# clementinboittiaux/sucre

Hardware: AMD Instinct MI355X
Metric: restored Mpixels/sec/GPU at 1080p, 64 neighbour views; % HBM roofline (higher is better)
Workload: dtype f32

## Files before the change

### sucre_amd/csrc/fit.hip

```cpp
#include <cstddef>
#include <type_traits>

#include "experiment.h"
#include "fit_math.h"
#include "handoff.h"

namespace sucre {

struct Water {
    float B[3], nb[3], ng[3];
};

template <class ParamAt>
__device__ __forceinline__ Water water_from(ParamAt param_at) {
    Water w;
#pragma unroll
    for (int c = 0; c < 3; ++c) {
        w.B[c] = param_at(c);
        w.nb[c] = -param_at(3 + c) * kLog2e;
        w.ng[c] = -param_at(6 + c) * kLog2e;
    }
    return w;
}
__device__ __forceinline__ Water load_water(const float *__restrict__ params) {
// ... 32 lines not shown
#pragma unroll
        for (int c = 0; c < 3; ++c) { e.a[j][c] = zz[j] * w.nb[c]; e.g[j][c] = zz[j] * w.ng[c]; }
    __builtin_amdgcn_sched_barrier(0);
#pragma unroll
    for (int j = 0; j < kGroupLv; ++j)
#pragma unroll
        for (int c = 0; c < 3; ++c) { e.a[j][c] = fast_exp2(e.a[j][c]); e.g[j][c] = fast_exp2(e.g[j][c]); }
    __builtin_amdgcn_sched_barrier(0);
}

__device__ __forceinline__ void grad_terms(float z, float a, float g, uint32_t k, bool valid, float Bc, float Jc, int c, Acc &acc) {
    const float omg = 1.0f - g;
    const float Ihat = __builtin_fmaf(Jc, a, Bc * omg);
    float r = __builtin_fmaf((float)k, kInv255, -Ihat);
    r = valid ? r : 0.0f;
    const float rz = r * z;
    acc.cost = __builtin_fmaf(r, r, acc.cost);
    acc.pa[c] = __builtin_fmaf(r, a, acc.pa[c]);
    acc.pb[c] = __builtin_fmaf(rz, a, acc.pb[c]);
    acc.sB[c] = __builtin_fmaf(r, omg, acc.sB[c]);
    acc.sGZ[c] = __builtin_fmaf(rz, g, acc.sGZ[c]);
}

template <bool kMasked>
__device__ __forceinline__ void accumulate_chunk(const float (&zz)[kGroupLv], const uint32_t (&cc)[3], const Water &w,
                                                 const float (&J)[3], Acc &acc) {
    if (kExpNoCompute) {
        acc.cost += (zz[0] + zz[1]) + (zz[2] + zz[3]) + (float)(cc[0] ^ cc[1] ^ cc[2]);
        return;
    }
    Exps e;
    chunk_exps(zz, w, e);
#pragma unroll
    for (int j = 0; j < kGroupLv; ++j) {
        const float z = zz[j];
        const bool valid = !kMasked || z > 0.0f;
#pragma unroll
        for (int c = 0; c < 3; ++c) grad_terms(z, e.a[j][c], e.g[j][c], (cc[c] >> (8 * j)) & 255u, valid, w.B[c], J[c], c, acc);
    }
}

__device__ __forceinline__ void accumulate_level(float z, const uint32_t (&k)[3], const Water &w, const float (&J)[3],
                                                 Acc &acc) {
    const bool valid = z > 0.0f;
#pragma unroll
    for (int c = 0; c < 3; ++c) grad_terms(z, fast_exp2(z * w.nb[c]), fast_exp2(z * w.ng[c]), k[c], valid, w.B[c], J[c], c, acc);
}

__device__ __forceinline__ float finite_or_zero(float x) { return __builtin_isfinite(x) ? x : 0.0f; }

struct AccOne {
    float q[9][3];
};

__device__ __forceinline__ void closed_terms(float z, float a, float g, uint32_t k, bool valid, float Bc, float Jp,
                                             float &q0, float &q1, float &q2, float &q3, float &q4, float &q5,
                                             float &q6, float &q7, float &q8) {
    const float omg = 1.0f - g;
    const float y = __builtin_fmaf((float)k, kInv255, -(Bc * omg));
    float p = __builtin_fmaf(-Jp, a, y);
    p = valid ? p : 0.0f;
    const float za = z * a, zg = z * g;
    q0 = __builtin_fmaf(p, a, q0);
    q1 = __builtin_fmaf(a, valid ? a : 0.0f, q1);
    q2 = __builtin_fmaf(p, omg, q2);
    q3 = __builtin_fmaf(a, omg, q3);
    q4 = __builtin_fmaf(p, za, q4);
    q5 = __builtin_fmaf(a, za, q5);
    q6 = __builtin_fmaf(p, zg, q6);
    q7 = __builtin_fmaf(a, zg, q7);
    q8 = __builtin_fmaf(p, p, q8);
}

template <bool kMasked>
__device__ __forceinline__ void accumulate_chunk(const float (&zz)[kGroupLv], const uint32_t (&cc)[3], const Water &w,
                                                 const float (&Jp)[3], AccOne &acc) {
    if (kExpNoCompute) {
        acc.q[8][0] += (zz[0] + zz[1]) + (zz[2] + zz[3]) + (float)(cc[0] ^ cc[1] ^ cc[2]);
        return;
    }
    Exps e;
    chunk_exps(zz, w, e);
#pragma unroll
    for (int j = 0; j < kGroupLv; ++j) {
        const float z = zz[j];
        const bool valid = !kMasked || z > 0.0f;
#pragma unroll
        for (int c = 0; c < 3; ++c)
            closed_terms(z, e.a[j][c], e.g[j][c], (cc[c] >> (8 * j)) & 255u, valid, w.B[c], Jp[c], acc.q[0][c], acc.q[1][c],
                         acc.q[2][c], acc.q[3][c], acc.q[4][c], acc.q[5][c], acc.q[6][c], acc.q[7][c], acc.q[8][c]);
    }
}

__device__ __forceinline__ void accumulate_level(float z, const uint32_t (&k)[3], const Water &w, const float (&Jp)[3],
                                                 AccOne &acc) {
    if (kExpNoCompute) {
        acc.q[8][0] += z + (float)(k[0] ^ k[1] ^ k[2]);
        return;
    }
    const bool valid = z > 0.0f;
#pragma unroll
    for (int c = 0; c < 3; ++c)
        closed_terms(z, fast_exp2(z * w.nb[c]), fast_exp2(z * w.ng[c]), k[c], valid, w.B[c], Jp[c], acc.q[0][c], acc.q[1][c],
                     acc.q[2][c], acc.q[3][c], acc.q[4][c], acc.q[5][c], acc.q[6][c], acc.q[7][c], acc.q[8][c]);
}

constexpr int kRing = SUCRE_RING;
constexpr int kAhead = kRing - 1;
constexpr int kSlot = 2048;

struct __attribute__((aligned(16))) FitLds {
    uint8_t ring[4][kRing][kSlot];
    double stot[kSumsPad];
    float wsum[4][kNumSums];
    double wtotal[4][kNumSums];
    int is_last, is_last_total;
};

__device__ __forceinline__ uint32_t lds_addr(const void *p) {
    return static_cast<uint32_t>(reinterpret_cast<uintptr_t>(p));
}

constexpr uint32_t kShapeFull = 1u << 31;
constexpr uint32_t kShapeTrail = 1u << 30;
__host__ __device__ constexpr uint32_t full_chunk_b(int fmt) { return (uint32_t)(chunk_bytes(fmt) - 1024) / 16u; }
__host__ __device__ __forceinline__ uint32_t item_shape(uint32_t bytes, bool full_chunk) {
    const uint32_t pieces = bytes / 16u;
// ... 12 lines not shown
        "s_mov_b32 %0, m0\n\t"
        "s_mov_b32 m0, %3\n\t"
        "s_nop 0\n\t"
        "global_load_lds_dwordx4 %1, %2" SUCRE_DMA_POLICY "\n\t"
        "s_mov_b32 m0, %4\n\t"
        "s_nop 0\n\t"
        "global_load_lds_dwordx4 %5, %2" SUCRE_DMA_POLICY "\n\t"
        "s_mov_b32 m0, %0"
        : "=&s"(keep)
        : "v"(voffA), "s"(src), "s"(slotA), "s"(slotB), "v"(voffB)
        : "memory");
}

__device__ __forceinline__ void wait_vm(uint32_t n) {
#define SUCRE_W(N) case N: asm volatile("s_waitcnt vmcnt(" #N ")" ::: "memory"); break;
    switch (n) {
        SUCRE_W(0) SUCRE_W(1) SUCRE_W(2) SUCRE_W(3) SUCRE_W(4) SUCRE_W(5) SUCRE_W(6) SUCRE_W(7) SUCRE_W(8) SUCRE_W(9)
        SUCRE_W(10) SUCRE_W(11) SUCRE_W(12) SUCRE_W(13) SUCRE_W(14) SUCRE_W(15) SUCRE_W(16) SUCRE_W(17) SUCRE_W(18)
        SUCRE_W(19) SUCRE_W(20) SUCRE_W(21)
        default: asm volatile("s_waitcnt vmcnt(0)" ::: "memory"); break;
    }
#undef SUCRE_W
}
static_assert(2 * kAhead + 9 <= 63, "s_waitcnt vmcnt takes six bits");

__device__ __forceinline__ uint32_t strip_items(uint32_t levels, int mode) { return 1u + ((levels + 3u) >> 2) + (mode == 0 ? 1u : 0u); }

__global__ __launch_bounds__(256) void plan_kernel(const StripMeta *__restrict__ meta, int n_strips, const uint32_t *__restrict__ store_fmt, uint32_t W0, uint32_t W1,
                                                   uint32_t Kmax, uint32_t stride0, uint32_t stride1, uint32_t kmax0, uint32_t kmax1,
                                                   PlanItem *__restrict__ plan0, PlanItem *__restrict__ plan1,
                                                   StripEntry *__restrict__ strips0, StripEntry *__restrict__ strips1,
                                                   uint32_t *__restrict__ count0, uint32_t *__restrict__ count1, uint64_t comp_off,
                                                   uint64_t state_off) {
    const int mode = blockIdx.y;
    const int fmt = (int)store_fmt[0];
    const uint32_t W = mode ? W1 : W0, stride = mode ? stride1 : stride0, kmax = mode ? kmax1 : kmax0;
    PlanItem *plan = mode ? plan1 : plan0;
    StripEntry *strips = mode ? strips1 : strips0;
    uint32_t *count = mode ? count1 : count0;
    const uint32_t idx = blockIdx.x * 256u + threadIdx.x;
    const uint32_t wid = idx / Kmax, k = idx - wid * Kmax;
    if (wid >= W) return;
    const DealShares sh = deal_shares(mode, W / 4u);
    uint32_t start = 0u, strip = 0u, strip0 = 0u;
    const uint32_t K = deal_walk(wid, W, (uint32_t)n_strips, sh, [&](uint32_t s) { return meta[s].levels; }, [&](uint32_t kk, uint32_t s) {
        if (kk == 0u) strip0 = s;
        if (kk < k) start += strip_items(meta[s].levels, mode);
        if (kk == k) strip = s;
    });
    if (k == 0u) count[wid] = K;
    if (k >= K) return;
    const StripMeta m = meta[strip];
    const uint32_t nfull = m.levels >> 2, r = m.levels & 3u;
    const uint32_t nu = min(nfull, m.full >> 2);
    const uint32_t lb = (uint32_t)level_bytes(fmt);
    const uint64_t st = state_off + (uint64_t)strip * (kStateFloats * 4);
    PlanItem *out = plan + (size_t)wid * stride + start;
    strips[(size_t)wid * kmax + k] = StripEntry{strip, strip_counts(nu, nfull - nu, r)};
    *out++ = PlanItem{(uint32_t)(st >> 6), item_shape(3u * kStripPx * 4u, false)};
    for (uint32_t g = 0; g < nfull; ++g)
        *out++ = PlanItem{(uint32_t)((comp_off + (m.lvoff + (uint64_t)g * kGroupLv) * lb) >> 6), item_shape((uint32_t)chunk_bytes(fmt), true)};
    if (r) *out++ = PlanItem{(uint32_t)((comp_off + (m.lvoff + (uint64_t)nfull * kGroupLv) * lb) >> 6), item_shape(r * lb, false)};
    if (mode == 0) *out++ = PlanItem{(uint32_t)((st + 3 * kStripPx * 4) >> 6), item_shape(6u * kStripPx * 4u, false)};
    if (k + 1u == K) {
        const uint64_t st0 = state_off + (uint64_t)strip0 * (kStateFloats * 4);
        for (int j = 0; j < kAhead + 1; ++j) *out++ = PlanItem{(uint32_t)(st0 >> 6), item_shape(3u * kStripPx * 4u, false) | kShapeTrail};
    }
}

typedef uint32_t ItemRegs __attribute__((ext_vector_type(2)));
typedef const __attribute__((address_space(4))) ItemRegs *ConstItems;

template <class T>
__device__ __forceinline__ T *uniform_ptr(T *p) {
    const uint64_t u = reinterpret_cast<uint64_t>(p);
    const uint32_t lo = __builtin_amdgcn_readfirstlane((uint32_t)u), hi = __builtin_amdgcn_readfirstlane((uint32_t)(u >> 32));
    return reinterpret_cast<T *>(((uint64_t)hi << 32) | lo);
}

template <class T>
__device__ __forceinline__ ConstItems const_items(const T *p) {
    static_assert(sizeof(T) == 8, "two dwords per entry");
    return (ConstItems)(reinterpret_cast<uintptr_t>(uniform_ptr(p)));
}

struct RangeCodes { bool z24, z26; uint32_t zoff, fullB; };

template <int kFmt>
__device__ __forceinline__ RangeCodes range_codes_of(uint32_t f0, uint32_t f1) {
// ... 32 lines not shown
            asm("v_mad_u32_u24 %0, %1, 1, %2" : "=v"(bits) : "v"(w[j]), "s"(rc.zoff));
            if (kZ26) bits += ((h >> (2 * j)) & 3u) << 24;
            zz[j] = __uint_as_float(bits);
            if (masked) zz[j] = (kZ26 ? bits != rc.zoff : (w[j] & 0xffffffu) != 0u) ? zz[j] : 0.0f;
        }
        cc[0] = __builtin_amdgcn_perm(a.y, a.x, 0x0c0c0703u) | __builtin_amdgcn_perm(b.y, b.x, 0x07030c0cu);
        cc[1] = c.x; cc[2] = c.y;
    };
    if (kFmt == 0 && rc.z26) return read_codes(std::true_type{});
    if (kFmt == 0 && rc.z24) return read_codes(std::false_type{});
    if (kFmt == 0) {
        const float4 z4 = *reinterpret_cast<const float4 *>(sp + lane * 16);
        zz[0] = z4.x; zz[1] = z4.y; zz[2] = z4.z; zz[3] = z4.w;
    } else {
        const uint2 q = *reinterpret_cast<const uint2 *>(sp + lane * 8);
        zz[0] = (float)(q.x & 0xffffu) * kMPerMm; zz[1] = (float)(q.x >> 16) * kMPerMm;
        zz[2] = (float)(q.y & 0xffffu) * kMPerMm; zz[3] = (float)(q.y >> 16) * kMPerMm;
    }
    const uint32_t *cp = reinterpret_cast<const uint32_t *>(sp + (kFmt ? 2 : 4) * kStripPx * kGroupLv) + 3 * lane;
    cc[0] = cp[0]; cc[1] = cp[1]; cc[2] = cp[2];
}

template <int kFmt>
__device__ __forceinline__ void read_level(const uint8_t *sp, int lane, uint32_t r, uint32_t j, float &z, uint32_t (&k)[3], const RangeCodes &rc) {
    const bool z24 = kFmt == 0 && (rc.z24 || rc.z26);
    if (z24) {
        const uint8_t *zp = sp + (lane * r + j) * 3u;
        uint32_t code = (uint32_t)zp[0] | ((uint32_t)zp[1] << 8) | ((uint32_t)zp[2] << 16);
        if (rc.z26) {
            const uint32_t f = (uint32_t)lane * r + j;
            code |= ((reinterpret_cast<const uint32_t *>(sp + 6u * kStripPx * r)[f >> 4] >> (2u * (f & 15u))) & 3u) << 24;
        }
        z = code ? __uint_as_float(code + rc.zoff) : 0.0f;
    } else if (kFmt == 0) z = reinterpret_cast<const float *>(sp)[lane * r + j];
    else z = (float)reinterpret_cast<const uint16_t *>(sp)[lane * r + j] * kMPerMm;
    const uint8_t *cb = sp + (z24 ? 3 : kFmt ? 2 : 4) * kStripPx * r;
#pragma unroll
    for (int c = 0; c < 3; ++c) k[c] = cb[c * kStripPx * r + lane * r + j];
}

template <int kFmt>
__device__ __forceinline__ void issue_item(const ItemRegs it, uint32_t ring0, uint32_t slot_off, const uint8_t *__restrict__ ws, int lane, uint32_t fullB) {
    const uint32_t lane16 = (uint32_t)lane * 16u;
    const uint32_t voffB_full = (64u + min((uint32_t)lane, fullB - 1u)) * 16u;
    const uint8_t *src = ws + ((uint64_t)it.x << 6);
    const uint32_t slot = ring0 + slot_off;
    if (it.y & kShapeFull) {
        dma_item(src, slot, slot + 1024u, lane16, voffB_full);
    } else {
        const uint32_t a_last = it.y & 127u, b_last = (it.y >> 8) & 127u, b_base = (it.y >> 16) & 127u;
        dma_item(src, slot, slot + ((a_last + 1u) << 4), min((uint32_t)lane, a_last) << 4, (b_base + min((uint32_t)lane, b_last)) << 4);
    }
}

struct NoChain { static constexpr bool kOn = false; };
struct StreamChain {
    static constexpr bool kOn = true;
    ItemRegs head[kAhead + 1], se0;
    bool next_on;
    ItemRegs next_head[kAhead];
    const uint8_t *next_ws;
// ... 182 lines not shown
                if (kStep && t < 64) water_step(lds.stot, pstate, n_obs_total, co, trace_row);
            }
        }
    }
}

template <bool kFused, bool kStep = kFused>
__device__ __forceinline__ void finish_launch(FitLds &lds, float (&s)[kNumSums], float *partials, const AdamCoef &co,
                                              unsigned *ticket, double *gpart, int n_groups, double *sums,
                                              float *pstate, const uint64_t *__restrict__ n_obs_total,
                                              double *trace_row) {
    const int t = threadIdx.x;
    const int lane = t & 63;
    const int wave = __builtin_amdgcn_readfirstlane(t >> 6);
    wave_sums(s);
    if (lane == 0) {
#pragma unroll
        for (int q = 0; q < kNumSums; ++q) lds.wsum[wave][q] = s[q];
    }
    finish_from_wave_sums<kFused, kStep>(lds, partials, co, ticket, gpart, n_groups, sums, pstate, n_obs_total, trace_row);
}

template <class Chain>
__device__ __forceinline__ void store_stepped(float *p, float v) {
    if (kStoreNt == 1 || (kStoreNt == 2 && Chain::kOn)) __builtin_nontemporal_store(v, p);
    else *p = v;
}

template <int kFmt, bool kPrimed = false, class Chain = NoChain>
__device__ __forceinline__ void grad_pass(FitLds &lds, const PlanItem *__restrict__ plan, const StripEntry *__restrict__ strips, uint32_t n_strips_wave,
                                          const uint8_t *__restrict__ ws, float *__restrict__ state, int wave, int lane,
                                          const Water &w, float gscale, const AdamCoef &co, Acc &acc, float (&sBeta)[3], const RangeCodes &rc,
                                          Chain *chain = nullptr) {
    float J[3] = {0.f, 0.f, 0.f};
    stream_strips<kFmt, 9, true, kPrimed, Chain>(
        lds, plan, strips, n_strips_wave, ws, wave, lane, rc.fullB,
        [&](const uint8_t *sp) {
            const float *f = reinterpret_cast<const float *>(sp);
#pragma unroll
            for (int c = 0; c < 3; ++c) { J[c] = f[c * kStripPx + lane]; acc.pa[c] = 0.f; acc.pb[c] = 0.f; }
        },
        [&](const uint8_t *sp, bool masked) {
            float zz[kGroupLv];
            uint32_t cc[3];
            read_chunk<kFmt>(sp, lane, zz, cc, rc, masked);
            if (masked) accumulate_chunk<true>(zz, cc, w, J, acc);
            else accumulate_chunk<false>(zz, cc, w, J, acc);
        },
        [&](const uint8_t *sp, uint32_t r) {
            for (uint32_t j = 0; j < r; ++j) {
                float z;
                uint32_t k[3];
                read_level<kFmt>(sp, lane, r, j, z, k, rc);
                accumulate_level(z, k, w, J, acc);
            }
        },
        [&](uint32_t strip, const uint8_t *sp) {
            const float *f = reinterpret_cast<const float *>(sp);
            float *st = state + (size_t)strip * kStateFloats;
#pragma unroll
            for (int c = 0; c < 3; ++c) {
                float Jc = J[c], m = f[c * kStripPx + lane], v = f[(3 + c) * kStripPx + lane];
                sBeta[c] += (acc.pb[c] == 0.0f) ? 0.0f : Jc * acc.pb[c];
                adam_update_J(Jc, m, v, gscale * acc.pa[c], co);
                if (kExpNoStore) {
                    asm volatile("" ::"v"(Jc), "v"(m), "v"(v));
                    continue;
                }
                store_stepped<Chain>(&st[c * kStripPx + lane], Jc);
                store_stepped<Chain>(&st[(3 + c) * kStripPx + lane], m);
                store_stepped<Chain>(&st[(6 + c) * kStripPx + lane], v);
            }
        },
        chain);
}

__device__ __forceinline__ void zero_acc(Acc &acc) {
#pragma unroll
    for (int c = 0; c < 3; ++c) { acc.pa[c] = 0.f; acc.pb[c] = 0.f; acc.sB[c] = 0.f; acc.sGZ[c] = 0.f; }
    acc.cost = 0.f;
}

constexpr uint32_t kExpWaveSlots = 8192;
__device__ unsigned long long g_exp_wave_times[5][kExpWaveTimes ? kExpWaveSlots : 1];
}
SUCRE_EXP_EXPORT int sucre_exp_wave_times(unsigned long long *out) {
    return (int)hipMemcpyFromSymbol(out, HIP_SYMBOL(sucre::g_exp_wave_times), sizeof(sucre::g_exp_wave_times));
}
namespace sucre {

template <bool kFused, int kFmt>
__global__ __launch_bounds__(256, kFitWaves) void fit_grad_kernel(const uint8_t *__restrict__ ws,
                                                       const PlanItem *__restrict__ plan, const StripEntry *__restrict__ plan_strips, const uint32_t *__restrict__ plan_count,
                                                       uint32_t plan_stride, uint32_t plan_kmax,
                                                       float *pstate, const uint64_t *__restrict__ n_obs_total,
// ... 14 lines not shown

    Acc acc;
    zero_acc(acc);
    if (!fmt_ok) acc.cost = __builtin_nanf("");
    float sBeta[3] = {0.f, 0.f, 0.f};
    if (kExpWaveTimes && lane == 0 && wid < kExpWaveSlots) g_exp_wave_times[0][wid] = wall_clock64();
    grad_pass<kFmt>(lds, plan + (size_t)wid * plan_stride, plan_strips + (size_t)wid * plan_kmax, n_mine, ws, state, wave, lane, w, gscale, co, acc, sBeta, rc);
    if (kExpWaveTimes && lane == 0 && wid < kExpWaveSlots) g_exp_wave_times[1][wid] = wall_clock64();

    float s[kNumSums];
    pack_sums(s, acc.sB, acc.sGZ, sBeta, acc.cost);
    finish_launch<kFused>(lds, s, partials, co, ticket, gpart, n_groups, sums, pstate, n_obs_total, trace_row);
    if (kExpWaveTimes && lane == 0 && wid < kExpWaveSlots) { g_exp_wave_times[2][wid] = exp_t_in; g_exp_wave_times[3][wid] = wall_clock64(); g_exp_wave_times[4][wid] = clock64() - exp_c_in; }
}

struct ClosedSums { float sB[3], sGZ[3], sBeta[3], cost; };

template <int kFmt, bool kJOnly, bool kPrimed = false, class Chain = NoChain>
__device__ __forceinline__ void closed_pass(FitLds &lds, const PlanItem *__restrict__ plan, const StripEntry *__restrict__ strips, uint32_t n_strips_wave,
                                            const uint8_t *__restrict__ ws, float *__restrict__ state, int wave, int lane,
                                            const Water &w, bool fmt_ok, ClosedSums &cs, const RangeCodes &rc, Chain *chain = nullptr) {
    AccOne acc;
    float Jp[3] = {0.f, 0.f, 0.f};
    stream_strips<kFmt, 3, false, kPrimed, Chain>(
        lds, plan, strips, n_strips_wave, ws, wave, lane, rc.fullB,
        [&](const uint8_t *sp) {
            const float *f = reinterpret_cast<const float *>(sp);
#pragma unroll
            for (int c = 0; c < 3; ++c) {
                Jp[c] = kJOnly ? 0.0f : finite_or_zero(f[c * kStripPx + lane]);
            }
#pragma unroll
            for (int q = 0; q < 9; ++q)
#pragma unroll
                for (int c = 0; c < 3; ++c) acc.q[q][c] = 0.f;
        },
        [&](const uint8_t *sp, bool masked) {
            float zz[kGroupLv];
            uint32_t cc[3];
            read_chunk<kFmt>(sp, lane, zz, cc, rc, masked);
            if (masked) accumulate_chunk<true>(zz, cc, w, Jp, acc);
            else accumulate_chunk<false>(zz, cc, w, Jp, acc);
        },
        [&](const uint8_t *sp, uint32_t r) {
            for (uint32_t j = 0; j < r; ++j) {
                float z;
                uint32_t k[3];
                read_level<kFmt>(sp, lane, r, j, z, k, rc);
                accumulate_level(z, k, w, Jp, acc);
            }
        },
        [&](uint32_t strip, const uint8_t *) {
            float *st = state + (size_t)strip * kStateFloats;
#pragma unroll
            for (int c = 0; c < 3; ++c) {
                const float N = acc.q[0][c], D = acc.q[1][c];
                const float dJ = N / D;
                const float Jc = fmt_ok ? Jp[c] + dJ : __builtin_nanf("");
                store_stepped<Chain>(&st[c * kStripPx + lane], Jc);
                if (!kJOnly && D != 0.0f) {
                    cs.sB[c] += __builtin_fmaf(-dJ, acc.q[3][c], acc.q[2][c]);
                    cs.sBeta[c] += Jc * __builtin_fmaf(-dJ, acc.q[5][c], acc.q[4][c]);
                    cs.sGZ[c] += __builtin_fmaf(-dJ, acc.q[7][c], acc.q[6][c]);
                    cs.cost += __builtin_fmaf(-dJ, N, acc.q[8][c]);
                } else if (!kJOnly && N != 0.0f) {
                    cs.sB[c] += dJ;
                    cs.sBeta[c] += dJ;
                    cs.sGZ[c] += dJ;
                    cs.cost += __builtin_inff();
                }
            }
        },
        chain);
}

template <bool kFused, int kFmt, bool kJOnly>
__global__ __launch_bounds__(256, kClosedWaves) void fit_closed_kernel(const uint8_t *__restrict__ ws,
                                                         const PlanItem *__restrict__ plan, const StripEntry *__restrict__ plan_strips, const uint32_t *__restrict__ plan_count,
                                                       uint32_t plan_stride, uint32_t plan_kmax,
                                                         float *pstate, const uint64_t *__restrict__ n_obs_total,
                                                         float *__restrict__ state, float *partials, const AdamCoef co,
                                                         unsigned *ticket, double *gpart, int n_groups, double *sums,
                                                         double *trace_row, const uint32_t *__restrict__ obs_format) {
    __shared__ FitLds lds;
    const int t = threadIdx.x;
    const int lane = t & 63;
    const int wave = __builtin_amdgcn_readfirstlane(t >> 6);
    const Water w = load_water_uniform(pstate);
    const RangeCodes rc = range_codes<kFmt>(obs_format);
    const bool fmt_ok = store_matches<kFmt>(obs_format);
    const uint32_t wid = blockIdx.x * 4u + (uint32_t)wave;
    const uint32_t n_mine = (fmt_ok || kJOnly) ? plan_count[wid] : 0u;
    ClosedSums cs = {{0.f, 0.f, 0.f}, {0.f, 0.f, 0.f}, {0.f, 0.f, 0.f}, fmt_ok ? 0.f : __builtin_nanf("")};
    if (kExpWaveTimes && !kJOnly && lane == 0 && wid < kExpWaveSlots) g_exp_wave_times[0][wid] = wall_clock64();
// ... 366 lines not shown
}

__global__ __launch_bounds__(64) void param_step_kernel(const double *__restrict__ sums, float *__restrict__ pstate,
                                                        const uint64_t *__restrict__ n_obs_total, const AdamCoef co,
                                                        double *__restrict__ trace_row) {
    water_step(sums, pstate, n_obs_total, co, trace_row);
}

__global__ __launch_bounds__(256) void fit_init_kernel(const uint8_t *__restrict__ rgb1,
                                                       const float *__restrict__ depth1,
                                                       const float *__restrict__ J0, int H, int W, int tiles_x,
                                                       const uint32_t *__restrict__ perm, float *__restrict__ state,
                                                       float *__restrict__ pstate,
                                                       unsigned *__restrict__ ticket, int n_tickets,
                                                       const Params9 p0) {
    const int tile = blockIdx.x, t = threadIdx.x;
    const uint32_t src = perm[(size_t)tile * kTilePx + t];
    const int stile = src / kTilePx, sslot = src % kTilePx;
    const int ty = stile / tiles_x, tx = stile - ty * tiles_x;
    const int v = ty * kTile + (sslot >> 4), u = tx * kTile + (sslot & 15);
    const bool inside = v < H && u < W;
    const size_t o = inside ? (size_t)v * W + u : 0;
    const bool valid = inside && !(depth1[o] <= 0.0f);
    float *st = state + ((size_t)tile * kStripsPerTile + (t >> 6)) * kStateFloats + (t & 63);
#pragma unroll
    for (int c = 0; c < 3; ++c) {
        float Jc = __builtin_nanf("");
        if (valid) Jc = J0 ? J0[o * 3 + c] : unit_from_u8(rgb1[o * 3 + c]);
        st[c * kStripPx] = Jc;
        st[(3 + c) * kStripPx] = 0.f;
        st[(6 + c) * kStripPx] = 0.f;
    }
    if (tile == 0 && t < 27) pstate[t] = t < 9 ? p0.v[t] : 0.f;
    for (int i = tile * 256 + t; i < n_tickets; i += gridDim.x * 256) ticket[i] = 0u;
}

__global__ __launch_bounds__(256) void export_J_kernel(const float *__restrict__ state, int H, int W, int tiles_x,
                                                       const uint32_t *__restrict__ invperm, float *__restrict__ J) {
    const int tile = blockIdx.x, t = threadIdx.x;
    const int ty = tile / tiles_x, tx = tile - ty * tiles_x;
    const int v = ty * kTile + (t >> 4), u = tx * kTile + (t & 15);
    if (v >= H || u >= W) return;
    const uint32_t dst = invperm[(size_t)tile * kTilePx + t];
    const size_t o = ((size_t)v * W + u) * 3;
    const float *st = state + (size_t)(dst / kStripPx) * kStateFloats + dst % kStripPx;
#pragma unroll
    for (int c = 0; c < 3; ++c) J[o + c] = st[c * kStripPx];
}

__global__ void set_n_obs_total_kernel(uint64_t *dst, uint64_t v) { *dst = v; }

hipError_t launch_fit_init(const Layout &L, uint8_t *ws, const uint8_t *rgb1, const float *depth1,
                           const float *params0, const float *J0, hipStream_t s) {
    hipLaunchKernelGGL(fit_init_kernel, dim3(L.n_tiles), dim3(256), 0, s, rgb1, depth1, J0, L.H, L.W, L.tiles_x,
                       reinterpret_cast<const uint32_t *>(ws + L.off_perm), reinterpret_cast<float *>(ws + L.off_state),
                       reinterpret_cast<float *>(ws + L.off_params),
                       reinterpret_cast<unsigned *>(ws + L.off_ticket), (1 + L.n_groups) * kTicketStride, params9(params0));
    return hipGetLastError();
}

template <class Kernel>
static void launch_fit_kernel(Kernel kernel, int mode, const Layout &L, uint8_t *ws, const AdamCoef &co, double *trace_row,
                              hipStream_t s) {
    hipLaunchKernelGGL(kernel, dim3(L.fit_blocks[mode]), dim3(256), 0, s, ws,
                       reinterpret_cast<const PlanItem *>(ws + L.off_plan[mode]),
                       reinterpret_cast<const StripEntry *>(ws + L.off_plan_strips[mode]),
                       reinterpret_cast<const uint32_t *>(ws + L.off_plan_count[mode]), (uint32_t)L.plan_stride[mode], (uint32_t)L.plan_kmax[mode],
                       reinterpret_cast<float *>(ws + L.off_params),
                       reinterpret_cast<const uint64_t *>(ws + L.off_n_obs_total),
                       reinterpret_cast<float *>(ws + L.off_state), reinterpret_cast<float *>(ws + L.off_partials), co,
// ... 177 lines not shown
```

### sucre_amd/csrc/fit_math.h

```cpp
#pragma once
#include "experiment.h"
#include "launch.h"

namespace sucre {

constexpr float kLog2e = 1.44269504088896340736f;
constexpr float kInv255Hi = (float)(1.0 / 255.0);
constexpr float kInv255Lo = (float)(1.0 / 255.0 - (double)kInv255Hi);

__device__ __forceinline__ float unit_from_u8(uint32_t k) {
    const float kf = (float)k;
    return __builtin_fmaf(kf, kInv255Hi, kf * kInv255Lo);
}

__device__ __forceinline__ float fast_exp2(float x) { return __builtin_amdgcn_exp2f(x); }

__device__ __forceinline__ float gradual_exp2(float x) {
    const bool tiny = x < -126.0f;
    return fast_exp2(tiny ? x + 64.0f : x) * (tiny ? 0x1p-64f : 1.0f);
}
template <bool kGradual>
__device__ __forceinline__ float exp2_as(float x) { return kGradual ? gradual_exp2(x) : fast_exp2(x); }

__device__ __forceinline__ void adam_update(float &p, float &m, float &v, float g, const AdamCoef &co) {
    m = __builtin_fmaf(co.w1, g - m, m);
    v = (v * co.beta2) + (co.w2 * g) * g;
    const float denom = sqrtf(v) / co.bc2_sqrt + co.eps;
    p = p + (co.step_size_neg * m) / denom;
}

template <class SumAt, class BAt>
__device__ __forceinline__ double water_grad(int q, float scale, SumAt sum_at, BAt B_at) {
    const int c = q % 3;
    if (q < 3) return -2.0 * (double)scale * sum_at(c);
    if (q < 6) return 2.0 * (double)scale * sum_at(6 + c);
    return -2.0 * (double)scale * (double)B_at(c) * sum_at(3 + c);
}

// ... 13 lines not shown
```

### sucre_amd/csrc/layout.h

```cpp
#pragma once
#include <stddef.h>
#include <stdint.h>

#include "experiment.h"

namespace sucre {

constexpr int kTile = 16;
constexpr int kTilePx = 256;
constexpr int kChunkZ = 1024;
constexpr int kChunkRGB = 768;
constexpr int kChunk = kChunkZ + kChunkRGB;
constexpr int kChunkZ16 = 512;
constexpr int kChunk16 = kChunkZ16 + kChunkRGB;
constexpr float kMmPerM = 1000.0f, kMPerMm = 0.001f;
constexpr int kStoreF32 = 0, kStoreU16 = 1, kStoreZ24 = 2, kStoreZ26 = 3;
constexpr int kChunk24 = 6 * 256;
constexpr int kChunk26 = kChunk24 + 64;
__host__ __device__ constexpr int chunk_bytes(int fmt) { return fmt == kStoreU16 ? kChunk16 : fmt == kStoreZ24 ? kChunk24 : fmt == kStoreZ26 ? kChunk26 : kChunk; }
__host__ __device__ constexpr uint32_t padded_levels(int fmt, uint32_t levels) { return fmt == kStoreZ26 ? (levels + 3u) & ~3u : levels; }
constexpr int kExtChunk = 3 * kChunkZ;
constexpr int kStripPx = 64;
constexpr int kStripsPerTile = kTilePx / kStripPx;
constexpr int kGroupLv = 4;
constexpr int kStateFloats = 9 * kStripPx;
__host__ __device__ constexpr int range_bytes(int fmt) { return fmt == kStoreU16 ? 2 : (fmt == kStoreZ24 || fmt == kStoreZ26) ? 3 : 4; }
__host__ __device__ constexpr int level_bytes(int fmt) { return (range_bytes(fmt) + 3) * kStripPx + (fmt == kStoreZ26 ? kStripPx / 4 : 0); }
static_assert(kGroupLv * level_bytes(kStoreZ26) == kChunk26 && kChunk26 % 64 == 0, "a 26-bit chunk is four levels and a whole number of 64-byte units");
constexpr int kExtLevelBytes = 3 * 4 * kStripPx;

struct StripMeta {
    uint64_t lvoff;
    uint32_t levels;
    uint32_t full;
};
constexpr int kNumSums = 10;
constexpr int kSumsPad = 12;
constexpr int kGroup = 32;
constexpr int kTicketStride = 16;
constexpr int kFitWaves = SUCRE_FIT_WAVES;
constexpr int kClosedWaves = SUCRE_CLOSED_WAVES;
constexpr int kFitGrid = 256 * kFitWaves;
constexpr int kClosedGrid = 256 * kClosedWaves;
constexpr int kMaxViews = 4096;
constexpr int kMinStripsPerWave = SUCRE_MIN_STRIPS;

constexpr uint32_t kDealDen = 64;
constexpr int kMaxGen = 8;
// ... 184 lines not shown
```

### sucre_amd/csrc/light.hip

```cpp
#include <cstddef>
#include <type_traits>
#include <mutex>
#include "fit_math.h"
#include "handoff.h"

namespace sucre {

constexpr int kLightSums = 19;
constexpr int kLightParams = 19;

struct LightLayout {
    size_t off_ext_dense, off_ext_comp;
    size_t off_params;
    size_t off_geom;
    size_t off_dexp;
    size_t off_partials;
    size_t off_sums;
    size_t off_deal;
    size_t off_ext2_dense, off_ext2_comp;
    size_t total;
};
constexpr uint32_t kLightMaxWaves = 8192;

static bool make_light_layout(const Layout &L, LightLayout *X, int ext_sets = 1) {
// ... 293 lines not shown
    constexpr float kInv255L = (float)(1.0 / 255.0);

    LightAcc acc;
#pragma unroll
    for (int q = 0; q < kLightSums; ++q) acc.s[q] = 0.f;

    const uint32_t W = (uint32_t)n_blocks * 4u, wid = blockIdx.x * 4u + (uint32_t)wave;
    const uint32_t n_mine = deal_count ? __builtin_amdgcn_readfirstlane(deal_count[wid]) : 0xffffffffu;
    for (uint32_t k = 0; k < n_mine; ++k) {
        uint32_t strip;
        if (deal_count) {
            strip = __builtin_amdgcn_readfirstlane(deal_strips[(size_t)wid * deal_kmax + k]);
        } else {
            strip = k * W + ((k & 1u) ? W - 1u - wid : wid);
            if (k * W >= (uint32_t)n_strips) break;
            if (strip >= (uint32_t)n_strips) continue;
        }
        const StripMeta sm = meta[strip];
        const uint32_t n = __builtin_amdgcn_readfirstlane(sm.levels), nch = (n + 3u) >> 2;
        const uint64_t lvoff = ((uint64_t)__builtin_amdgcn_readfirstlane((uint32_t)(sm.lvoff >> 32)) << 32) | __builtin_amdgcn_readfirstlane((uint32_t)sm.lvoff);
        const uint8_t *sobs = comp + lvoff * (uint64_t)level_bytes(0);
        const uint8_t *sext = ext + lvoff * (uint64_t)kExtLevelBytes;
        const uint8_t *sext2 = kBoth ? ext2 + lvoff * (uint64_t)kExtLevelBytes : nullptr;
        float *st = state + (size_t)strip * kStateFloats + lane;
        float J[3];
        if (kClosed) {
            float num[3], den[3];
            auto solve = [&](auto gradual) {
                constexpr bool kGradual = decltype(gradual)::value;
#pragma unroll
                for (int c = 0; c < 3; ++c) num[c] = den[c] = 0.f;
                auto load1 = [&](uint32_t g) { return load_light_chunk<kJOnly>(sobs, sext, g, min((uint32_t)kGroupLv, n - g * kGroupLv), lane); };
                auto solve_chunk = [&](const LightChunk &kk, uint32_t g) {
                    ColourChunk fc;
                    if (kBoth) fc = load_colour_chunk(sext2, g, min((uint32_t)kGroupLv, n - g * kGroupLv), lane);
                    if (kExpNoCompute) {
                        num[0] += chunk_checksum(kk);
                        den[0] = den[1] = den[2] = 1.0f;
                        return;
                    }
#pragma unroll
                    for (int j = 0; j < 4; ++j) {
                        if (!(kk.zz[j] > 0.0f)) continue;
                        const float cP[3] = {kk.xx[j], kk.yy[j], kk.ww[j]};
                        LightObs o;
                        if (kColour) { o.l = 1.0f; o.z = kk.zz[j]; }
                        else o = light_obs<kGradual>(cP, kk.zz[j], R, tl, M);
// ... 10 lines not shown
                if constexpr (kPingPong) {
                    LightChunk ka = nch ? load1(0) : LightChunk{}, kb2 = LightChunk{};
                    for (uint32_t g = 0; g < nch; g += 2u) {
                        if (g + 1u < nch) kb2 = load1(g + 1u);
                        solve_chunk(ka, g);
                        if (g + 1u < nch) {
                            if (g + 2u < nch) ka = load1(g + 2u);
                            solve_chunk(kb2, g + 1u);
                        }
                    }
                } else {
                    for (uint32_t g = 0; g < nch; ++g) solve_chunk(load1(g), g);
                }
            };
            solve(std::false_type{});
            const bool zero = den[0] == 0.f || den[1] == 0.f || den[2] == 0.f;
            if (n > 0 && __any(zero)) {
                const LightChunk k0 = load_light_chunk<false>(sobs, sext, 0, min((uint32_t)kGroupLv, n), lane);
                if (__any(zero && k0.zz[0] > 0.0f)) solve(std::true_type{});
            }
#pragma unroll
            for (int c = 0; c < 3; ++c) {
                J[c] = num[c] / den[c];
                st[c * kStripPx] = J[c];
            }
            if (kJOnly) continue;
        } else {
#pragma unroll
            for (int c = 0; c < 3; ++c) J[c] = st[c * kStripPx];
        }
        float pa[3] = {0.f, 0.f, 0.f}, pb[3] = {0.f, 0.f, 0.f};
        const float bJ[3] = {beta[0] * J[0], beta[1] * J[1], beta[2] * J[2]};
        auto chunk_at = [&](uint32_t i) { return kClosed ? nch - 1u - i : i; };
        auto levels_of = [&](uint32_t g) { return min((uint32_t)kGroupLv, n - g * kGroupLv); };
        constexpr bool kNoZ = !kClosed && !kColour && !kBoth;
        auto load_at = [&](uint32_t i) { return load_light_chunk<true, kNoZ>(sobs, sext, chunk_at(i), levels_of(chunk_at(i)), lane); };
        auto grad_chunk = [&](const LightChunk &kk, uint32_t gi) {
            ColourChunk fc;
            if (kBoth) fc = load_colour_chunk(sext2, chunk_at(gi), levels_of(chunk_at(gi)), lane);
            if (kExpNoCompute) {
                acc.s[9] += chunk_checksum(kk);
                return;
            }
#pragma unroll
            for (int j = 0; j < 4; ++j) {
                if (kNoZ ? kk.zz[j] == 0.0f : !(kk.zz[j] > 0.0f)) continue;
                const float cP[3] = {kk.xx[j], kk.yy[j], kk.ww[j]};
                LightObs o;
                if (kColour) { o.l = 1.0f; o.z = kk.zz[j]; }
                else o = light_obs(cP, kNoZ ? __builtin_amdgcn_sqrtf(__builtin_fmaf(cP[2], cP[2], __builtin_fmaf(cP[1], cP[1], cP[0] * cP[0]))) : kk.zz[j], R, tl, M);
                const float l = o.l, z = o.z;
                float dl = 0.f, dz = 0.f;
// ... 34 lines not shown
                acc.s[17] = __builtin_fmaf(k0, o.lp1, acc.s[17]);
                acc.s[18] = __builtin_fmaf(kf * o.lp1, o.lp1, acc.s[18]);
            }
        };
        if constexpr (kPingPong) {
            LightChunk ka = nch ? load_at(0) : LightChunk{}, kb2 = LightChunk{};
            for (uint32_t gi = 0; gi < nch; gi += 2u) {
                if (gi + 1u < nch) kb2 = load_at(gi + 1u);
                grad_chunk(ka, gi);
                if (gi + 1u < nch) {
                    if (gi + 2u < nch) ka = load_at(gi + 2u);
                    grad_chunk(kb2, gi + 1u);
                }
            }
        } else {
            LightChunk kn = nch ? load_at(0) : LightChunk{};
            for (uint32_t gi = 0; gi < nch; ++gi) {
                const LightChunk kk = kn;
                if (gi + 1u < nch) kn = load_at(gi + 1u);
                grad_chunk(kk, gi);
            }
        }
#pragma unroll
        for (int c = 0; c < 3; ++c) {
            if (kClosed) {
                acc.s[6 + c] += (pb[c] == 0.0f) ? 0.0f : J[c] * pb[c];
            } else {
                float Jc = J[c], m = st[(3 + c) * kStripPx], v = st[(6 + c) * kStripPx];
                acc.s[6 + c] += (pb[c] == 0.0f) ? 0.0f : Jc * pb[c];
                adam_update_J(Jc, m, v, gscale * pa[c], co);
                st[c * kStripPx] = Jc; st[(3 + c) * kStripPx] = m; st[(6 + c) * kStripPx] = v;
            }
        }
    }
    if (kJOnly) return;
#pragma unroll
    for (int q = 0; q < kLightSums; ++q) {
        const float x = wave_sum_lane0(acc.s[q]);
        if (lane == 0) wsum[wave][q] = x;
    }
    __syncthreads();
    if (t < kLightSums) partials[(size_t)t * n_blocks + blockIdx.x] = ((wsum[0][t] + wsum[1][t]) + wsum[2][t]) + wsum[3][t];
}

__global__ __launch_bounds__(256) void light_tail_kernel(const float *partials, int n_blocks, double *sums, float *pstate,
                                                         float *geom, double *dexp, const uint64_t *__restrict__ n_obs_total,
                                                         const AdamCoef co, double *trace_row) {
    __shared__ LightLds lds;
    light_reduce(partials, n_blocks, lds.sums, lds.w4);
    if (threadIdx.x < kLightSums) sums[threadIdx.x] = lds.sums[threadIdx.x];
    light_step(lds, pstate, geom, dexp, n_obs_total, co, trace_row);
}

struct LightParams19 { float v[kLightParams]; };

// ... 275 lines not shown
```

Before: 82.15.

## Interleave per-pixel state channels and batch exp work in level tails

Changes the per-strip state layout from channel-planar to per-pixel RGB triples, so each state plane (J, Adam m, Adam v) is written with one 12-byte vector store per lane instead of three scalar stores. The vmcnt budgets for stores drop accordingly. Separately, the remainder-level tail loop is specialised for 1-3 levels: exponents are computed in batches and colour loads are hoisted behind sched barriers to overlap latency. The risk is unaligned 3-wide stores splitting into partial transactions, plus extra code size from the templated tail variants.

```diff
diff --git a/sucre_amd/csrc/fit.hip b/sucre_amd/csrc/fit.hip
--- a/sucre_amd/csrc/fit.hip
+++ b/sucre_amd/csrc/fit.hip
@@ -78,30 +78,10 @@
     acc.sGZ[c] = __builtin_fmaf(rz, g, acc.sGZ[c]);
 }
 
-template <bool kMasked>
-__device__ __forceinline__ void accumulate_chunk(const float (&zz)[kGroupLv], const uint32_t (&cc)[3], const Water &w,
-                                                 const float (&J)[3], Acc &acc) {
-    if (kExpNoCompute) {
-        acc.cost += (zz[0] + zz[1]) + (zz[2] + zz[3]) + (float)(cc[0] ^ cc[1] ^ cc[2]);
-        return;
-    }
-    Exps e;
-    chunk_exps(zz, w, e);
-#pragma unroll
-    for (int j = 0; j < kGroupLv; ++j) {
-        const float z = zz[j];
-        const bool valid = !kMasked || z > 0.0f;
-#pragma unroll
-        for (int c = 0; c < 3; ++c) grad_terms(z, e.a[j][c], e.g[j][c], (cc[c] >> (8 * j)) & 255u, valid, w.B[c], J[c], c, acc);
-    }
-}
-
-__device__ __forceinline__ void accumulate_level(float z, const uint32_t (&k)[3], const Water &w, const float (&J)[3],
-                                                 Acc &acc) {
-    const bool valid = z > 0.0f;
-#pragma unroll
-    for (int c = 0; c < 3; ++c) grad_terms(z, fast_exp2(z * w.nb[c]), fast_exp2(z * w.ng[c]), k[c], valid, w.B[c], J[c], c, acc);
-}
+__device__ __forceinline__ void obs_terms(float z, float a, float g, uint32_t k, bool valid, const Water &w, const float (&J)[3], int c, Acc &acc) {
+    grad_terms(z, a, g, k, valid, w.B[c], J[c], c, acc);
+}
+__device__ __forceinline__ float &checksum_of(Acc &acc) { return acc.cost; }
 
 __device__ __forceinline__ float finite_or_zero(float x) { return __builtin_isfinite(x) ? x : 0.0f; }
 
@@ -128,11 +108,16 @@
     q8 = __builtin_fmaf(p, p, q8);
 }
 
-template <bool kMasked>
+__device__ __forceinline__ void obs_terms(float z, float a, float g, uint32_t k, bool valid, const Water &w, const float (&Jp)[3], int c, AccOne &acc) {
+    closed_terms(z, a, g, k, valid, w.B[c], Jp[c], acc.q[0][c], acc.q[1][c], acc.q[2][c], acc.q[3][c], acc.q[4][c], acc.q[5][c], acc.q[6][c], acc.q[7][c], acc.q[8][c]);
+}
+__device__ __forceinline__ float &checksum_of(AccOne &acc) { return acc.q[8][0]; }
+
+template <bool kMasked, class A>
 __device__ __forceinline__ void accumulate_chunk(const float (&zz)[kGroupLv], const uint32_t (&cc)[3], const Water &w,
-                                                 const float (&Jp)[3], AccOne &acc) {
+                                                 const float (&J)[3], A &acc) {
     if (kExpNoCompute) {
-        acc.q[8][0] += (zz[0] + zz[1]) + (zz[2] + zz[3]) + (float)(cc[0] ^ cc[1] ^ cc[2]);
+        checksum_of(acc) += (zz[0] + zz[1]) + (zz[2] + zz[3]) + (float)(cc[0] ^ cc[1] ^ cc[2]);
         return;
     }
     Exps e;
@@ -142,23 +127,37 @@
         const float z = zz[j];
         const bool valid = !kMasked || z > 0.0f;
 #pragma unroll
-        for (int c = 0; c < 3; ++c)
-            closed_terms(z, e.a[j][c], e.g[j][c], (cc[c] >> (8 * j)) & 255u, valid, w.B[c], Jp[c], acc.q[0][c], acc.q[1][c],
-                         acc.q[2][c], acc.q[3][c], acc.q[4][c], acc.q[5][c], acc.q[6][c], acc.q[7][c], acc.q[8][c]);
-    }
-}
-
-__device__ __forceinline__ void accumulate_level(float z, const uint32_t (&k)[3], const Water &w, const float (&Jp)[3],
-                                                 AccOne &acc) {
+        for (int c = 0; c < 3; ++c) obs_terms(z, e.a[j][c], e.g[j][c], (cc[c] >> (8 * j)) & 255u, valid, w, J, c, acc);
+    }
+}
+
+template <int kR, class Colours, class A>
+__device__ __forceinline__ void accumulate_short(const float (&z)[kR], Colours colours, const Water &w, const float (&J)[3], A &acc) {
+    uint32_t k[kR][3];
     if (kExpNoCompute) {
-        acc.q[8][0] += z + (float)(k[0] ^ k[1] ^ k[2]);
+#pragma unroll
+        for (int j = 0; j < kR; ++j) { colours(j, k[j]); checksum_of(acc) += z[j] + (float)(k[j][0] ^ k[j][1] ^ k[j][2]); }
         return;
     }
-    const bool valid = z > 0.0f;
-#pragma unroll
-    for (int c = 0; c < 3; ++c)
-        closed_terms(z, fast_exp2(z * w.nb[c]), fast_exp2(z * w.ng[c]), k[c], valid, w.B[c], Jp[c], acc.q[0][c], acc.q[1][c],
-                     acc.q[2][c], acc.q[3][c], acc.q[4][c], acc.q[5][c], acc.q[6][c], acc.q[7][c], acc.q[8][c]);
+    float a[kR][3], g[kR][3];
+#pragma unroll
+    for (int j = 0; j < kR; ++j)
+#pragma unroll
+        for (int c = 0; c < 3; ++c) { a[j][c] = z[j] * w.nb[c]; g[j][c] = z[j] * w.ng[c]; }
+    __builtin_amdgcn_sched_barrier(0);
+#pragma unroll
+    for (int j = 0; j < kR; ++j) colours(j, k[j]);
+#pragma unroll
+    for (int j = 0; j < kR; ++j)
+#pragma unroll
+        for (int c = 0; c < 3; ++c) { a[j][c] = fast_exp2(a[j][c]); g[j][c] = fast_exp2(g[j][c]); }
+    __builtin_amdgcn_sched_barrier(0);
+#pragma unroll
+    for (int j = 0; j < kR; ++j) {
+        const bool valid = z[j] > 0.0f;
+#pragma unroll
+        for (int c = 0; c < 3; ++c) obs_terms(z[j], a[j][c], g[j][c], k[j][c], valid, w, J, c, acc);
+    }
 }
 
 constexpr int kRing = SUCRE_RING;
@@ -217,7 +216,8 @@
     }
 #undef SUCRE_W
 }
-static_assert(2 * kAhead + 9 <= 63, "s_waitcnt vmcnt takes six bits");
+constexpr int kGradStores = kExpNoStore ? 0 : 3, kClosedStores = 1;
+static_assert(2 * kAhead + kGradStores <= 63 && 2 * kAhead + kClosedStores <= 63, "s_waitcnt vmcnt takes six bits");
 
 __device__ __forceinline__ uint32_t strip_items(uint32_t levels, int mode) { return 1u + ((levels + 3u) >> 2) + (mode == 0 ? 1u : 0u); }
 
@@ -252,14 +252,14 @@
     const uint64_t st = state_off + (uint64_t)strip * (kStateFloats * 4);
     PlanItem *out = plan + (size_t)wid * stride + start;
     strips[(size_t)wid * kmax + k] = StripEntry{strip, strip_counts(nu, nfull - nu, r)};
-    *out++ = PlanItem{(uint32_t)(st >> 6), item_shape(3u * kStripPx * 4u, false)};
+    *out++ = PlanItem{(uint32_t)(st >> 6), item_shape(kPlaneFloats * 4u, false)};
     for (uint32_t g = 0; g < nfull; ++g)
         *out++ = PlanItem{(uint32_t)((comp_off + (m.lvoff + (uint64_t)g * kGroupLv) * lb) >> 6), item_shape((uint32_t)chunk_bytes(fmt), true)};
     if (r) *out++ = PlanItem{(uint32_t)((comp_off + (m.lvoff + (uint64_t)nfull * kGroupLv) * lb) >> 6), item_shape(r * lb, false)};
-    if (mode == 0) *out++ = PlanItem{(uint32_t)((st + 3 * kStripPx * 4) >> 6), item_shape(6u * kStripPx * 4u, false)};
+    if (mode == 0) *out++ = PlanItem{(uint32_t)((st + state_at(kStateAvg, 0, 0) * 4) >> 6), item_shape(2u * kPlaneFloats * 4u, false)};
     if (k + 1u == K) {
         const uint64_t st0 = state_off + (uint64_t)strip0 * (kStateFloats * 4);
-        for (int j = 0; j < kAhead + 1; ++j) *out++ = PlanItem{(uint32_t)(st0 >> 6), item_shape(3u * kStripPx * 4u, false) | kShapeTrail};
+        for (int j = 0; j < kAhead + 1; ++j) *out++ = PlanItem{(uint32_t)(st0 >> 6), item_shape(kPlaneFloats * 4u, false) | kShapeTrail};
     }
 }
 
@@ -338,21 +338,40 @@
 }
 
 template <int kFmt>
-__device__ __forceinline__ void read_level(const uint8_t *sp, int lane, uint32_t r, uint32_t j, float &z, uint32_t (&k)[3], const RangeCodes &rc) {
-    const bool z24 = kFmt == 0 && (rc.z24 || rc.z26);
-    if (z24) {
+__device__ __forceinline__ float read_level_z(const uint8_t *sp, int lane, uint32_t r, uint32_t j, const RangeCodes &rc) {
+    if (kFmt == 0 && (rc.z24 || rc.z26)) {
         const uint8_t *zp = sp + (lane * r + j) * 3u;
         uint32_t code = (uint32_t)zp[0] | ((uint32_t)zp[1] << 8) | ((uint32_t)zp[2] << 16);
         if (rc.z26) {
             const uint32_t f = (uint32_t)lane * r + j;
             code |= ((reinterpret_cast<const uint32_t *>(sp + 6u * kStripPx * r)[f >> 4] >> (2u * (f & 15u))) & 3u) << 24;
         }
-        z = code ? __uint_as_float(code + rc.zoff) : 0.0f;
-    } else if (kFmt == 0) z = reinterpret_cast<const float *>(sp)[lane * r + j];
-    else z = (float)reinterpret_cast<const uint16_t *>(sp)[lane * r + j] * kMPerMm;
+        return code ? __uint_as_float(code + rc.zoff) : 0.0f;
+    }
+    if (kFmt == 0) return reinterpret_cast<const float *>(sp)[lane * r + j];
+    return (float)reinterpret_cast<const uint16_t *>(sp)[lane * r + j] * kMPerMm;
+}
+template <int kFmt>
+__device__ __forceinline__ void read_level_k(const uint8_t *sp, int lane, uint32_t r, uint32_t j, uint32_t (&k)[3], const RangeCodes &rc) {
+    const bool z24 = kFmt == 0 && (rc.z24 || rc.z26);
     const uint8_t *cb = sp + (z24 ? 3 : kFmt ? 2 : 4) * kStripPx * r;
 #pragma unroll
     for (int c = 0; c < 3; ++c) k[c] = cb[c * kStripPx * r + lane * r + j];
+}
+
+template <int kFmt, class A>
+__device__ __forceinline__ void accumulate_tail(const uint8_t *sp, int lane, uint32_t r, const Water &w, const float (&J)[3], A &acc, const RangeCodes &rc) {
+    asm volatile("" : "+v"(lane));
+    auto body = [&](auto n) {
+        constexpr int kR = decltype(n)::value;
+        float z[kR];
+#pragma unroll
+        for (int j = 0; j < kR; ++j) z[j] = read_level_z<kFmt>(sp, lane, (uint32_t)kR, (uint32_t)j, rc);
+        accumulate_short<kR>(z, [&](int j, uint32_t (&k)[3]) { read_level_k<kFmt>(sp, lane, (uint32_t)kR, (uint32_t)j, k, rc); }, w, J, acc);
+    };
+    if (r == 1u) body(std::integral_constant<int, 1>{});
+    else if (r == 2u) body(std::integral_constant<int, 2>{});
+    else body(std::integral_constant<int, 3>{});
 }
 
 template <int kFmt>
@@ -581,9 +600,8 @@
 }
 
 template <class Chain>
-__device__ __forceinline__ void store_stepped(float *p, float v) {
-    if (kStoreNt == 1 || (kStoreNt == 2 && Chain::kOn)) __builtin_nontemporal_store(v, p);
-    else *p = v;
+__device__ __forceinline__ void store_stepped(float *st, int plane, int lane, const float (&x)[3]) {
+    store_triple<kStoreNt == 1 || (kStoreNt == 2 && Chain::kOn)>(st, plane, lane, x);
 }
 
 template <int kFmt, bool kPrimed = false, class Chain = NoChain>
@@ -592,12 +610,12 @@
                                           const Water &w, float gscale, const AdamCoef &co, Acc &acc, float (&sBeta)[3], const RangeCodes &rc,
                                           Chain *chain = nullptr) {
     float J[3] = {0.f, 0.f, 0.f};
-    stream_strips<kFmt, 9, true, kPrimed, Chain>(
+    stream_strips<kFmt, kGradStores, true, kPrimed, Chain>(
         lds, plan, strips, n_strips_wave, ws, wave, lane, rc.fullB,
         [&](const uint8_t *sp) {
-            const float *f = reinterpret_cast<const float *>(sp);
-#pragma unroll
-            for (int c = 0; c < 3; ++c) { J[c] = f[c * kStripPx + lane]; acc.pa[c] = 0.f; acc.pb[c] = 0.f; }
+            read_triple_lds(sp, kStateJ, kStateJ, lane, J);
+#pragma unroll
+            for (int c = 0; c < 3; ++c) { acc.pa[c] = 0.f; acc.pb[c] = 0.f; }
         },
         [&](const uint8_t *sp, bool masked) {
             float zz[kGroupLv];
@@ -606,30 +624,25 @@
             if (masked) accumulate_chunk<true>(zz, cc, w, J, acc);
             else accumulate_chunk<false>(zz, cc, w, J, acc);
         },
-        [&](const uint8_t *sp, uint32_t r) {
-            for (uint32_t j = 0; j < r; ++j) {
-                float z;
-                uint32_t k[3];
-                read_level<kFmt>(sp, lane, r, j, z, k, rc);
-                accumulate_level(z, k, w, J, acc);
+        [&](const uint8_t *sp, uint32_t r) { accumulate_tail<kFmt>(sp, lane, r, w, J, acc, rc); },
+        [&](uint32_t strip, const uint8_t *sp) {
+            float *st = state + (size_t)strip * kStateFloats;
+            float m[3], v[3];
+            read_triple_lds(sp, kStateAvg, kStateAvg, lane, m);
+            read_triple_lds(sp, kStateAvg, kStateAvgSq, lane, v);
+#pragma unroll
+            for (int c = 0; c < 3; ++c) {
+                sBeta[c] += (acc.pb[c] == 0.0f) ? 0.0f : J[c] * acc.pb[c];
+                adam_update_J(J[c], m[c], v[c], gscale * acc.pa[c], co);
             }
-        },
-        [&](uint32_t strip, const uint8_t *sp) {
-            const float *f = reinterpret_cast<const float *>(sp);
-            float *st = state + (size_t)strip * kStateFloats;
-#pragma unroll
-            for (int c = 0; c < 3; ++c) {
-                float Jc = J[c], m = f[c * kStripPx + lane], v = f[(3 + c) * kStripPx + lane];
-                sBeta[c] += (acc.pb[c] == 0.0f) ? 0.0f : Jc * acc.pb[c];
-                adam_update_J(Jc, m, v, gscale * acc.pa[c], co);
-                if (kExpNoStore) {
-                    asm volatile("" ::"v"(Jc), "v"(m), "v"(v));
-                    continue;
-                }
-                store_stepped<Chain>(&st[c * kStripPx + lane], Jc);
-                store_stepped<Chain>(&st[(3 + c) * kStripPx + lane], m);
-                store_stepped<Chain>(&st[(6 + c) * kStripPx + lane], v);
+            if (kExpNoStore) {
+#pragma unroll
+                for (int c = 0; c < 3; ++c) asm volatile("" ::"v"(J[c]), "v"(m[c]), "v"(v[c]));
+                return;
             }
+            store_stepped<Chain>(st, kStateJ, lane, J);
+            store_stepped<Chain>(st, kStateAvg, lane, m);
+            store_stepped<Chain>(st, kStateAvgSq, lane, v);
         },
         chain);
 }
@@ -690,13 +703,13 @@
                                             const Water &w, bool fmt_ok, ClosedSums &cs, const RangeCodes &rc, Chain *chain = nullptr) {
     AccOne acc;
     float Jp[3] = {0.f, 0.f, 0.f};
-    stream_strips<kFmt, 3, false, kPrimed, Chain>(
+    stream_strips<kFmt, kClosedStores, false, kPrimed, Chain>(
         lds, plan, strips, n_strips_wave, ws, wave, lane, rc.fullB,
         [&](const uint8_t *sp) {
-            const float *f = reinterpret_cast<const float *>(sp);
+            read_triple_lds(sp, kStateJ, kStateJ, lane, Jp);
 #pragma unroll
             for (int c = 0; c < 3; ++c) {
-                Jp[c] = kJOnly ? 0.0f : finite_or_zero(f[c * kStripPx + lane]);
+                Jp[c] = kJOnly ? 0.0f : finite_or_zero(Jp[c]);
             }
 #pragma unroll
             for (int q = 0; q < 9; ++q)
@@ -710,22 +723,16 @@
             if (masked) accumulate_chunk<true>(zz, cc, w, Jp, acc);
             else accumulate_chunk<false>(zz, cc, w, Jp, acc);
         },
-        [&](const uint8_t *sp, uint32_t r) {
-            for (uint32_t j = 0; j < r; ++j) {
-                float z;
-                uint32_t k[3];
-                read_level<kFmt>(sp, lane, r, j, z, k, rc);
-                accumulate_level(z, k, w, Jp, acc);
-            }
-        },
+        [&](const uint8_t *sp, uint32_t r) { accumulate_tail<kFmt>(sp, lane, r, w, Jp, acc, rc); },
         [&](uint32_t strip, const uint8_t *) {
             float *st = state + (size_t)strip * kStateFloats;
+            float Jn[3];
 #pragma unroll
             for (int c = 0; c < 3; ++c) {
                 const float N = acc.q[0][c], D = acc.q[1][c];
                 const float dJ = N / D;
                 const float Jc = fmt_ok ? Jp[c] + dJ : __builtin_nanf("");
-                store_stepped<Chain>(&st[c * kStripPx + lane], Jc);
+                Jn[c] = Jc;
                 if (!kJOnly && D != 0.0f) {
                     cs.sB[c] += __builtin_fmaf(-dJ, acc.q[3][c], acc.q[2][c]);
                     cs.sBeta[c] += Jc * __builtin_fmaf(-dJ, acc.q[5][c], acc.q[4][c]);
@@ -738,6 +745,7 @@
                     cs.cost += __builtin_inff();
                 }
             }
+            store_stepped<Chain>(st, kStateJ, lane, Jn);
         },
         chain);
 }
@@ -1150,15 +1158,17 @@
     const bool inside = v < H && u < W;
     const size_t o = inside ? (size_t)v * W + u : 0;
     const bool valid = inside && !(depth1[o] <= 0.0f);
-    float *st = state + ((size_t)tile * kStripsPerTile + (t >> 6)) * kStateFloats + (t & 63);
+    float *st = state + ((size_t)tile * kStripsPerTile + (t >> 6)) * kStateFloats;
+    float J[3];
+    const float zero[3] = {0.f, 0.f, 0.f};
 #pragma unroll
     for (int c = 0; c < 3; ++c) {
-        float Jc = __builtin_nanf("");
-        if (valid) Jc = J0 ? J0[o * 3 + c] : unit_from_u8(rgb1[o * 3 + c]);
-        st[c * kStripPx] = Jc;
-        st[(3 + c) * kStripPx] = 0.f;
-        st[(6 + c) * kStripPx] = 0.f;
-    }
+        J[c] = __builtin_nanf("");
+        if (valid) J[c] = J0 ? J0[o * 3 + c] : unit_from_u8(rgb1[o * 3 + c]);
+    }
+    store_triple(st, kStateJ, t & 63, J);
+    store_triple(st, kStateAvg, t & 63, zero);
+    store_triple(st, kStateAvgSq, t & 63, zero);
     if (tile == 0 && t < 27) pstate[t] = t < 9 ? p0.v[t] : 0.f;
     for (int i = tile * 256 + t; i < n_tickets; i += gridDim.x * 256) ticket[i] = 0u;
 }
@@ -1171,9 +1181,10 @@
     if (v >= H || u >= W) return;
     const uint32_t dst = invperm[(size_t)tile * kTilePx + t];
     const size_t o = ((size_t)v * W + u) * 3;
-    const float *st = state + (size_t)(dst / kStripPx) * kStateFloats + dst % kStripPx;
-#pragma unroll
-    for (int c = 0; c < 3; ++c) J[o + c] = st[c * kStripPx];
+    float Jp[3];
+    load_triple(state + (size_t)(dst / kStripPx) * kStateFloats, kStateJ, (int)(dst % kStripPx), Jp);
+#pragma unroll
+    for (int c = 0; c < 3; ++c) J[o + c] = Jp[c];
 }
 
 __global__ void set_n_obs_total_kernel(uint64_t *dst, uint64_t v) { *dst = v; }
diff --git a/sucre_amd/csrc/fit_math.h b/sucre_amd/csrc/fit_math.h
--- a/sucre_amd/csrc/fit_math.h
+++ b/sucre_amd/csrc/fit_math.h
@@ -14,6 +14,25 @@
 }
 
 __device__ __forceinline__ float fast_exp2(float x) { return __builtin_amdgcn_exp2f(x); }
+
+typedef float Triple __attribute__((ext_vector_type(3), aligned(4)));
+
+__device__ __forceinline__ void load_triple(const float *block, int plane, int lane, float (&x)[3]) {
+    const Triple t = *reinterpret_cast<const Triple *>(block + state_at(plane, 0, lane));
+    x[0] = t.x; x[1] = t.y; x[2] = t.z;
+}
+template <bool kNt = false>
+__device__ __forceinline__ void store_triple(float *block, int plane, int lane, const float (&x)[3]) {
+    const Triple t = {x[0], x[1], x[2]};
+    Triple *p = reinterpret_cast<Triple *>(block + state_at(plane, 0, lane));
+    if (kNt) __builtin_nontemporal_store(t, p);
+    else *p = t;
+}
+__device__ __forceinline__ void read_triple_lds(const uint8_t *slot, int first, int plane, int lane, float (&x)[3]) {
+    const float *f = reinterpret_cast<const float *>(slot);
+#pragma unroll
+    for (int c = 0; c < 3; ++c) x[c] = f[state_at(plane - first, c, lane)];
+}
 
 __device__ __forceinline__ float gradual_exp2(float x) {
     const bool tiny = x < -126.0f;
diff --git a/sucre_amd/csrc/layout.h b/sucre_amd/csrc/layout.h
--- a/sucre_amd/csrc/layout.h
+++ b/sucre_amd/csrc/layout.h
@@ -23,7 +23,10 @@
 constexpr int kStripPx = 64;
 constexpr int kStripsPerTile = kTilePx / kStripPx;
 constexpr int kGroupLv = 4;
-constexpr int kStateFloats = 9 * kStripPx;
+constexpr int kStateJ = 0, kStateAvg = 1, kStateAvgSq = 2;
+constexpr int kPlaneFloats = 3 * kStripPx;
+constexpr int kStateFloats = 3 * kPlaneFloats;
+__host__ __device__ constexpr int state_at(int plane, int c, int lane) { return plane * kPlaneFloats + 3 * lane + c; }
 __host__ __device__ constexpr int range_bytes(int fmt) { return fmt == kStoreU16 ? 2 : (fmt == kStoreZ24 || fmt == kStoreZ26) ? 3 : 4; }
 __host__ __device__ constexpr int level_bytes(int fmt) { return (range_bytes(fmt) + 3) * kStripPx + (fmt == kStoreZ26 ? kStripPx / 4 : 0); }
 static_assert(kGroupLv * level_bytes(kStoreZ26) == kChunk26 && kChunk26 % 64 == 0, "a 26-bit chunk is four levels and a whole number of 64-byte units");
diff --git a/sucre_amd/csrc/light.hip b/sucre_amd/csrc/light.hip
--- a/sucre_amd/csrc/light.hip
+++ b/sucre_amd/csrc/light.hip
@@ -339,7 +339,7 @@
         const uint8_t *sobs = comp + lvoff * (uint64_t)level_bytes(0);
         const uint8_t *sext = ext + lvoff * (uint64_t)kExtLevelBytes;
         const uint8_t *sext2 = kBoth ? ext2 + lvoff * (uint64_t)kExtLevelBytes : nullptr;
-        float *st = state + (size_t)strip * kStateFloats + lane;
+        float *st = state + (size_t)strip * kStateFloats;
         float J[3];
         if (kClosed) {
             float num[3], den[3];
@@ -396,12 +396,11 @@
 #pragma unroll
             for (int c = 0; c < 3; ++c) {
                 J[c] = num[c] / den[c];
-                st[c * kStripPx] = J[c];
             }
+            store_triple(st, kStateJ, lane, J);
             if (kJOnly) continue;
         } else {
-#pragma unroll
-            for (int c = 0; c < 3; ++c) J[c] = st[c * kStripPx];
+            load_triple(st, kStateJ, lane, J);
         }
         float pa[3] = {0.f, 0.f, 0.f}, pb[3] = {0.f, 0.f, 0.f};
         const float bJ[3] = {beta[0] * J[0], beta[1] * J[1], beta[2] * J[2]};
@@ -482,15 +481,16 @@
             }
         }
 #pragma unroll
-        for (int c = 0; c < 3; ++c) {
-            if (kClosed) {
-                acc.s[6 + c] += (pb[c] == 0.0f) ? 0.0f : J[c] * pb[c];
-            } else {
-                float Jc = J[c], m = st[(3 + c) * kStripPx], v = st[(6 + c) * kStripPx];
-                acc.s[6 + c] += (pb[c] == 0.0f) ? 0.0f : Jc * pb[c];
-                adam_update_J(Jc, m, v, gscale * pa[c], co);
-                st[c * kStripPx] = Jc; st[(3 + c) * kStripPx] = m; st[(6 + c) * kStripPx] = v;
-            }
+        for (int c = 0; c < 3; ++c) acc.s[6 + c] += (pb[c] == 0.0f) ? 0.0f : J[c] * pb[c];
+        if (!kClosed) {
+            float m[3], v[3];
+            load_triple(st, kStateAvg, lane, m);
+            load_triple(st, kStateAvgSq, lane, v);
+#pragma unroll
+            for (int c = 0; c < 3; ++c) adam_update_J(J[c], m[c], v[c], gscale * pa[c], co);
+            store_triple(st, kStateJ, lane, J);
+            store_triple(st, kStateAvg, lane, m);
+            store_triple(st, kStateAvgSq, lane, v);
         }
     }
     if (kJOnly) return;
```

Measured after the change: 81.87. No clear change (-0.3%).
